# wyhuai/DDNM

Hardware: AMD Instinct MI355X
Metric: restored images/sec @256×256, 100 DDIM steps, 4×SR; 1/2/4/8 GPU (higher is better)
Workload: dtype f32 (3x3 convolutions: fp32 operands carried as hi + lo fp16 halves, three fp16 MFMA products per product, fp32 accumulate -- operand error 2^-22, measured closer to fp64 than the fp32 MFMA kernel; everything else fp32); 1 GPU; celeba_hq.yml SVD sr_bicubic 4x, sigma_y=0, eta=0.85, T_sampling=100, batch_size=8 per GPU (BASELINE configs[1]); global_batch=8, image=3x256x256, parallelism=dp1 (image sharding)

## Files before the change

ddnm_amd/_lib.py:

```python
import ctypes
import os
from ctypes import POINTER, Structure, c_char_p, c_float, c_int32, c_int64, c_uint8, c_uint32, c_void_p

_HERE = os.path.dirname(os.path.abspath(__file__))
LIB_PATH = os.path.join(_HERE, "libddnm_hip.so")

c_f32p = c_void_p


class ConvDesc(Structure):
    _fields_ = [
        ("src0", c_void_p), ("src1", c_void_p), ("weight", c_void_p), ("bias", c_void_p),
        ("badd", c_void_p), ("res", c_void_p), ("gn_scale", c_void_p), ("gn_shift", c_void_p),
        ("out", c_void_p),
        ("B", c_int32), ("Hin", c_int32), ("Win", c_int32),
        ("C0", c_int32), ("C1", c_int32), ("Cout", c_int32),
        ("ksize", c_int32), ("stride", c_int32), ("pad", c_int32),
        ("Ho", c_int32), ("Wo", c_int32),
        ("ups", c_int32), ("gn_silu", c_int32), ("out_nchw", c_int32),
        ("badd_stride", c_int32), ("tile", c_int32),
        ("workspace", c_void_p), ("workspace_floats", c_int64),
        ("res_ups", c_int32), ("src_f16", c_int32),
        ("stats_out", c_void_p),
        ("skip0", c_void_p), ("skip1", c_void_p), ("skip_weight", c_void_p),
# ... 32 lines not shown
        ("fin_gamma", c_void_p), ("fin_beta", c_void_p), ("fin_film", c_void_p),
        ("fin_scale", c_void_p), ("fin_shift", c_void_p),
        ("fin_eps", c_float), ("fin_film_stride", c_int32), ("fin_groups", c_int32), ("reserved2", c_int32),
    ]


class StepScalars(Structure):
    _fields_ = [("sqrt_1m_at", c_float), ("sqrt_at", c_float), ("sqrt_at_next", c_float),
                ("c1", c_float), ("c2", c_float), ("lam", c_float),
                ("rng_on", c_uint32), ("rng_seed_lo", c_uint32), ("rng_seed_hi", c_uint32), ("rng_iter", c_uint32),
                ("rng_image_base", c_uint32), ("reserved_rng", c_uint32)]


PROTOTYPES = {
    "ddnm_version": (c_int32, []),
    "ddnm_error_string": (c_char_p, [c_int32]),
    "ddnm_build_digest": (c_char_p, []),
    "ddnm_sizeof": (c_int32, [c_int32]),
    "ddnm_conv2d_f32": (c_int32, [POINTER(ConvDesc), c_void_p]),
    "ddnm_conv3x3_small_cout_f32": (c_int32, [POINTER(ConvDesc), c_void_p]),
    "ddnm_conv3x3_small_cout_f32_supported": (c_int32, [POINTER(ConvDesc)]),
    "ddnm_conv2d_f32_tile_n": (c_int32, [POINTER(ConvDesc)]),
    "ddnm_conv2d_f32_workspace_floats": (c_int64, [POINTER(ConvDesc)]),
    "ddnm_conv2d_f32_stats_tiles": (c_int32, [POINTER(ConvDesc)]),
    "ddnm_conv2d_f32_fuses_skip": (c_int32, [POINTER(ConvDesc)]),
    "ddnm_spectral_mix_f32": (c_int32, [c_void_p, c_void_p, c_void_p, c_int64, c_void_p, c_int64, c_float, c_float, c_float,
                                        c_float, c_int32, c_void_p]),
    "ddnm_hq_x0_f32": (c_int32, [c_void_p, c_void_p, c_int64, c_void_p, c_int32, c_int64, c_float, c_float, c_int32,
                                 c_void_p]),
    "ddnm_hq_project_f32": (c_int32, [c_void_p, c_void_p, c_void_p, c_void_p, c_int64, c_float, c_void_p]),
    "ddnm_copy_rect_f32": (c_int32, [c_void_p, c_int32, c_int32, c_int32, c_int32, c_void_p, c_int32, c_int32, c_int32,
                                     c_int32, c_int32, c_int32, c_int32, c_void_p]),
    "ddnm_hq_sample_f32": (c_int32, [c_void_p, c_void_p, c_void_p, c_void_p, c_void_p, c_int64, c_float, c_float, c_float,
                                     c_float, c_void_p]),
    "ddnm_patchify_f32": (c_int32, [c_void_p, c_void_p, c_int32, c_int32, c_int32, c_int32, c_void_p]),
    "ddnm_im2col3x3_f16": (c_int32, [c_void_p, c_void_p, c_void_p, c_void_p, c_void_p, c_int32, c_int32, c_int32, c_int32,
                                     c_int32, c_int32, c_void_p]),
    "ddnm_gn_apply_f16": (c_int32, [c_void_p, c_void_p, c_void_p, c_void_p, c_void_p, c_int32, c_int32, c_int32, c_int32,
                                    c_int32, c_void_p]),
    "ddnm_gn_finalize_tiles_f32": (c_int32, [c_void_p, c_int32, c_int32, c_void_p, c_int32, c_int32, c_void_p, c_void_p,
                                             c_int32, c_int32, c_int32, c_float, c_void_p, c_void_p, c_void_p, c_int32,
                                             c_void_p, c_void_p]),
    "ddnm_gn_finalize_tiles_amax_f32": (c_int32, [c_void_p, c_int32, c_int32, c_void_p, c_int32, c_int32, c_void_p, c_void_p,
                                                  c_int32, c_int32, c_int32, c_float, c_void_p, c_void_p, c_void_p, c_int32,
                                                  c_void_p, c_void_p, c_void_p]),
    "ddnm_amax_bound_f32": (c_int32, [c_void_p, c_int64, c_int32, c_void_p, c_int64, c_int32, c_void_p, c_int32, c_void_p]),
    "ddnm_conv3x3_f16_f32": (c_int32, [POINTER(ConvDesc), c_void_p]),
    "ddnm_conv3x3_f16_supported": (c_int32, [POINTER(ConvDesc)]),
    "ddnm_conv3x3_f16_workspace_floats": (c_int64, [POINTER(ConvDesc)]),
    "ddnm_conv3x3_f16_stats_tiles": (c_int32, [POINTER(ConvDesc)]),
    "ddnm_conv3x3_s16_f32": (c_int32, [POINTER(ConvDesc), c_void_p]),
    "ddnm_conv3x3_s16_supported": (c_int32, [POINTER(ConvDesc)]),
    "ddnm_conv3x3_s16_persistent": (c_int32, [POINTER(ConvDesc)]),
    "ddnm_conv3x3_s16_ups_subpixel_supported": (c_int32, [POINTER(ConvDesc)]),
    "ddnm_conv3x3_s16_workspace_floats": (c_int64, [POINTER(ConvDesc)]),
    "ddnm_conv3x3_s16_stats_tiles": (c_int32, [POINTER(ConvDesc)]),
    "ddnm_conv3x3_s16_act_scale": (c_float, []),
    "ddnm_conv_gather_s16_f32": (c_int32, [POINTER(ConvDesc), c_void_p]),
    "ddnm_conv_gather_s16_supported": (c_int32, [POINTER(ConvDesc)]),
    "ddnm_conv_gather_s16_workspace_floats": (c_int64, [POINTER(ConvDesc)]),
    "ddnm_conv_gather_s16_stats_tiles": (c_int32, [POINTER(ConvDesc)]),
    "ddnm_conv_gather_s16_gemm1x1": (c_int32, [POINTER(ConvDesc)]),
    "ddnm_conv_gather_s16_wslice": (c_int32, [POINTER(ConvDesc)]),
    "ddnm_conv16": (c_int32, [POINTER(Conv16Desc), c_void_p]),
    "ddnm_conv16_supported": (c_int32, [POINTER(Conv16Desc)]),
    "ddnm_conv16_fuses_fin": (c_int32, [POINTER(Conv16Desc)]),
    "ddnm_conv16_workspace_floats": (c_int64, [POINTER(Conv16Desc)]),
    "ddnm_conv16_stats_tiles": (c_int32, [POINTER(Conv16Desc)]),
    "ddnm_gn_apply_h16": (c_int32, [c_void_p, c_void_p, c_void_p, c_void_p, c_void_p, c_int32, c_int32, c_int32, c_int32,
                                    c_int32, c_int32, c_int32, c_void_p]),
    "ddnm_im2col3x3_h16": (c_int32, [c_void_p, c_void_p, c_void_p, c_void_p, c_void_p, c_int32, c_int32, c_int32, c_int32,
                                     c_int32, c_int32, c_void_p]),
    "ddnm_nchw_to_nhwc_h16": (c_int32, [c_void_p, c_void_p, c_int32, c_int32, c_int32, c_int32, c_void_p]),
    "ddnm_gn_stats_h16": (c_int32, [c_void_p, c_void_p, c_int32, c_int32, c_int32, c_int32, c_void_p]),
    "ddnm_attn16_d64": (c_int32, [c_void_p, c_void_p, c_int32, c_int32, c_int32, c_void_p]),
    "ddnm_conv1x1_f16_f32": (c_int32, [POINTER(ConvDesc), c_void_p]),
    "ddnm_conv1x1_f16_supported": (c_int32, [POINTER(ConvDesc)]),
    "ddnm_conv1x1_f16_workspace_floats": (c_int64, [POINTER(ConvDesc)]),
    "ddnm_conv1x1_f16_stats_tiles": (c_int32, [POINTER(ConvDesc)]),
    "ddnm_gn_stats_f32": (c_int32, [c_void_p, c_void_p, c_int32, c_int32, c_int32, c_int32, c_int32, c_void_p,
                                    c_int32, c_void_p]),
    "ddnm_gn_nchunk": (c_int32, [c_int32, c_int32]),
    "ddnm_gn_finalize_f32": (c_int32, [c_void_p, c_int32, c_void_p, c_void_p, c_int32, c_int32, c_int32, c_int32,
                                       c_float, c_void_p, c_void_p, c_void_p, c_int32, c_void_p, c_void_p]),
    "ddnm_bgemm_f32": (c_int32, [POINTER(GemmDesc), c_void_p]),
    "ddnm_gn_bwd_f32": (c_int32, [c_void_p, c_void_p, c_int32, c_void_p, c_void_p, c_void_p, c_int32, c_void_p, c_int32,
                                  c_int32, c_int32, c_int32, c_int32, c_int32, c_void_p, c_int32, c_void_p, c_void_p,
                                  c_void_p]),
    "ddnm_gn_bwd_nchunk": (c_int32, [c_int32, c_int32]),
    "ddnm_gn_bwd_h16": (c_int32, [c_void_p, c_void_p, c_int32, c_void_p, c_void_p, c_void_p, c_int32, c_void_p, c_int32,
                                  c_int32, c_int32, c_int32, c_int32, c_int32, c_void_p, c_int32, c_void_p, c_void_p,
                                  c_void_p]),
    "ddnm_pool_tokens_h16": (c_int32, [c_void_p, c_void_p, c_void_p, c_void_p, c_void_p, c_int32, c_int32, c_int32,
                                       c_void_p]),
    "ddnm_pool_tokens_bwd_h16": (c_int32, [c_void_p, c_void_p, c_int32, c_int32, c_int32, c_void_p]),
    "ddnm_attn16_d64_lse": (c_int32, [c_void_p, c_void_p, c_void_p, c_int32, c_int32, c_int32, c_void_p]),
    "ddnm_attn16_d64_bwd": (c_int32, [c_void_p, c_void_p, c_void_p, c_void_p, c_void_p, c_void_p, c_int32, c_int32,
                                      c_int32, c_void_p]),
    "ddnm_softmax_bwd_rows_f32": (c_int32, [c_void_p, c_void_p, c_int64, c_int32, c_int32, c_float, c_void_p]),
    "ddnm_pool_tokens_f32": (c_int32, [c_void_p, c_void_p, c_void_p, c_void_p, c_void_p, c_int32, c_int32, c_int32,
                                       c_void_p]),
    "ddnm_pool_attn_fwd_f32": (c_int32, [c_void_p, c_void_p, c_void_p, c_int32, c_int32, c_int32, c_int32, c_void_p]),
    "ddnm_pool_attn_bwd_f32": (c_int32, [c_void_p, c_void_p, c_void_p, c_void_p, c_int32, c_int32, c_int32, c_int32,
                                         c_void_p]),
    "ddnm_pool_tokens_bwd_f32": (c_int32, [c_void_p, c_void_p, c_int32, c_int32, c_int32, c_void_p]),
    "ddnm_logsoftmax_grad_f32": (c_int32, [c_void_p, c_void_p, c_void_p, c_int32, c_int32, c_void_p]),
# ... 170 lines not shown
```

ddnm_amd/build.py:

```python
import hashlib
import os
import shutil
import subprocess
import sys

HERE = os.path.dirname(os.path.abspath(__file__))
CSRC = os.path.join(HERE, "csrc")
LIB = os.path.join(HERE, "libddnm_hip.so")
STAMP = os.path.join(HERE, ".libddnm_hip.stamp")
OBJ = os.path.join(HERE, "_obj")
SOURCES = ["conv_igemm_f32.hip", "conv_igemm_f16.hip", "conv_s16_persist.hip", "conv_s16_subpixel.hip", "conv_gather_s16.hip", "conv1x1_s16.hip", "conv_s16_wslice.hip", "conv_small_f32.hip", "conv1x1_f16.hip", "conv16.hip", "act16.hip", "attn16.hip", "attn_d512.hip", "attn16_bwd.hip", "gemm_f32.hip", "groupnorm.hip", "misc.hip", "ddnm_step.hip", "fwht.hip", "backward.hip", "metrics.hip"]
FLAGS = ["--offload-arch=gfx950", "-O3", "-std=c++17", "-fPIC", "-shared", "-Wall", "-Wno-unused-function"]


def _hipcc():
    for c in (os.environ.get("HIPCC"), shutil.which("hipcc"), "/opt/rocm/bin/hipcc"):
        if c and os.path.exists(c):
            return c
    raise RuntimeError("hipcc not found (set HIPCC)")


def _digest():
    h = hashlib.sha256()
    for f in sorted(os.listdir(CSRC)) + ["../../include/ddnm_hip.h"]:
        with open(os.path.join(CSRC, f), "rb") as fh:
            h.update(f.encode() + fh.read())
    h.update(" ".join(FLAGS).encode())
    return h.hexdigest()


LAST_BUILD = {"compiled": False}


def build(force=False, verbose=False):
    dig = _digest()
    LAST_BUILD["compiled"] = False
    if not force and os.path.exists(LIB) and os.path.exists(STAMP) and open(STAMP).read() == dig:
        return LIB
    LAST_BUILD["compiled"] = True
    tmp = LIB + f".tmp{os.getpid()}"
    os.makedirs(OBJ, exist_ok=True)
    hh = hashlib.sha256()
    for f in sorted(os.listdir(CSRC)) + ["../../include/ddnm_hip.h"]:
        if f.endswith(".h"):
            with open(os.path.join(CSRC, f), "rb") as fh:
                hh.update(f.encode() + fh.read())
    hh.update(" ".join(FLAGS).encode())
    cflags = [f for f in FLAGS if f != "-shared"]
    jobs, objs = [], []
    for s in SOURCES:
        h = hashlib.sha256(hh.digest())
        with open(os.path.join(CSRC, s), "rb") as fh:
            h.update(fh.read())
        extra = [f'-DDDNM_BUILD_DIGEST="{dig}"'] if s == "misc.hip" else []
        h.update(" ".join(extra).encode())
        obj = os.path.join(OBJ, f"{s}.{h.hexdigest()[:16]}.o")
        objs.append(obj)
        if force or not os.path.exists(obj):
            jobs.append((s, [_hipcc()] + cflags + extra + ["-c", os.path.join(CSRC, s), "-o", obj + f".tmp{os.getpid()}"], obj))
    if jobs:
        from concurrent.futures import ThreadPoolExecutor

        def run(job):
            s, cmd, obj = job
# ... 34 lines not shown
```

ddnm_amd/csrc/conv_common.h:

```cpp
#pragma once
#include "common.h"

struct ConvArgs {
    ddnm_conv_desc d;
    int Cin, ntaps, Hs, Ws;
    int m_tiles, n_tiles;
    int tiles_x;
    int TW, TW_log2;
    int ksplit;
    float* ws;
};

static inline bool conv_operand_offsets_fit(const ddnm_conv_desc* d) {
    const int64_t px = (int64_t)d->B * (d->ups ? d->Hin / 2 : d->Hin) * (d->ups ? d->Win / 2 : d->Win);
    const int64_t cmax = d->C0 > d->C1 ? d->C0 : d->C1;
    return px * cmax * (d->src_f16 ? 2 : 4) < (int64_t)1 << 31;
}
static inline bool conv_sizes_addressable(const ddnm_conv_desc* d) {
    const int64_t lim = (int64_t)1 << 31;
    const int64_t out_el = (int64_t)d->B * d->Ho * d->Wo * d->Cout;
    const int64_t cout_pad = ((int64_t)d->Cout + 127) / 128 * 128;
    const int64_t w_b = cout_pad * d->ksize * d->ksize * ((int64_t)d->C0 + d->C1) * 4;
    const int64_t sk_el = (int64_t)d->B * d->Ho * d->Wo * (d->SC0 > d->SC1 ? d->SC0 : d->SC1);
    return out_el < lim && conv_operand_offsets_fit(d) && w_b < lim && sk_el < lim;
}

bool conv3x3_s16_persist_eligible(const ConvArgs& p);
int conv3x3_s16_persist_launch(const ConvArgs& p, hipStream_t s);
bool conv3x3_s16_ups_subpixel_ok(const ddnm_conv_desc* d);
int conv3x3_s16_ups_subpixel_run(const ddnm_conv_desc* d, hipStream_t s);
bool conv1x1_s16_routes(const ddnm_conv_desc* d, int plan_ksplit, int plan_bm);
int conv1x1_s16_launch(const ddnm_conv_desc* d, int plan_ksplit, int plan_bm, int run_ksplit, hipStream_t s);
bool conv3x3_s16_wslice_routes(const ddnm_conv_desc* d, int plan_ksplit, int plan_bm);
int conv3x3_s16_wslice_launch(const ddnm_conv_desc* d, int ksplit, hipStream_t s);
int conv_persist_grid_cus();

struct TileMap {
    int img, ty0, tx0, th_unused, TW, TW_log2, flat_base, Wo;
    bool two_d;
    __device__ __forceinline__ void pixel(int r, int& oy, int& ox) const {
        if (two_d) {
            oy = ty0 + (r >> TW_log2);
            ox = tx0 + (r & (TW - 1));
        } else {
            const int pix = flat_base + r;
            oy = pix / Wo;
            ox = pix - oy * Wo;
        }
    }
};

template <int BM>
__device__ __forceinline__ TileMap make_tilemap(const ConvArgs& p, int m_tile) {
    TileMap t;
    const int HWo = p.d.Ho * p.d.Wo;
    const int per_img = HWo / BM;
    t.img = m_tile / per_img;
    const int t_in_img = m_tile - t.img * per_img;
    t.TW = p.TW;
    t.TW_log2 = p.TW_log2;
    t.Wo = p.d.Wo;
    t.two_d = p.tiles_x != 0;
    if (t.two_d) {
        const int ty = t_in_img / p.tiles_x, tx = t_in_img - ty * p.tiles_x;
        t.ty0 = ty * (BM >> p.TW_log2);
        t.tx0 = tx << p.TW_log2;
        t.flat_base = 0;
    } else {
        t.ty0 = t.tx0 = 0;
        t.flat_base = t_in_img * BM;
    }
    return t;
}

template <int WM, int WN, int MT, int NT, bool RES_ALL_UPFRONT = false>
__device__ __forceinline__ void conv_epilogue(const ConvArgs& p, const TileMap& tm, int n_tile, int m_tile, int slice,
                                              f32x16 (&acc)[MT][NT], float* lds, const float acc_scale = 1.f) {
    constexpr int BN = WN * NT * 32;
    const ddnm_conv_desc& d = p.d;
    const int lane = threadIdx.x & 63, wave = threadIdx.x >> 6;
    const int wm = wave / WN, wn = wave % WN;
    const int ncol = lane & 31, rsel = 4 * (lane >> 5);
    const bool partial = p.ksplit > 1;
    float* __restrict__ ws = partial ? p.ws + (size_t)slice * d.B * d.Ho * d.Wo * d.Cout : nullptr;
    const float* __restrict__ res = d.res;
    float* __restrict__ out = d.out;
    const bool want_stats = d.stats_out != nullptr && !partial;
// ... 314 lines not shown
```

ddnm_amd/csrc/conv_igemm_f16.hip:

```cpp
#include "s16_tile.h"

constexpr int KC16 = 64;
constexpr int F16_BM = 256;
constexpr int F16_KS_TARGET = 256;
constexpr int LDH = KC16 + 8;

template <int WM, int WN, int MT, int NT, bool SRC16, bool SPLIT = false, bool ASCALE = false>
__global__ __launch_bounds__(WM * WN * 64, 1) void conv3x3_halo_f16_kernel(const ConvArgs p) {
    static_assert(!(SPLIT && SRC16), "the split form reads fp32 activations");
    static_assert(SPLIT || !ASCALE, "operand scaling belongs to the split form");
    constexpr int NTHREADS = WM * WN * 64;
    constexpr int BM = WM * MT * 32, BN = WN * NT * 32;
    constexpr int MAXH = BM == 512 ? 612 : (BM == 256 ? 340 : (BM == 128 ? 204 : 136));
    constexpr int KCH = SPLIT ? KC16 / 2 : KC16;
    constexpr int WE = SPLIT ? 2 : 1;
    constexpr int HVEC = SRC16 ? 8 : 4;
    constexpr int HCOLS = KCH / HVEC;
    constexpr int HROWS_PER_PASS = NTHREADS / HCOLS;
    constexpr int HR = (MAXH + HROWS_PER_PASS - 1) / HROWS_PER_PASS;
    static_assert(KC16 == 64, "an LDS weight row is 128 bytes");
    constexpr int BCOLS = 8;
    constexpr int BROWS_PER_PASS = NTHREADS / BCOLS;
    constexpr int BR = BN / BROWS_PER_PASS;
    static_assert(BR >= 1 && BN % BROWS_PER_PASS == 0, "weight tile / thread mapping");
// ... 281 lines not shown
    int tw = 32;
    while (tw > 8 && (d->Wo % tw || d->Ho % (pl->BM / tw))) tw >>= 1;
    if (d->Wo % tw || d->Ho % (pl->BM / tw)) return false;
    pl->TW = tw;
    pl->TW_log2 = tw == 32 ? 5 : (tw == 16 ? 4 : 3);
    pl->tiles_x = d->Wo / tw;
    const long tiles = (long)d->B * (HWo / pl->BM) * (d->Cout / 128);
    int ks = 1;
    const int nchunks = Cin / kch;
    if (tiles < 192) {
        ks = (int)((F16_KS_TARGET + tiles - 1) / tiles);
        if (ks > nchunks) ks = nchunks;
        if (ks > 16) ks = 16;
    }
    pl->ksplit = ks;
    return true;
}

extern "C" int ddnm_conv3x3_f16_supported(const ddnm_conv_desc* d) {
    PlanF16 pl;
    return d && plan_f16(d, &pl) ? 1 : 0;
}

extern "C" int64_t ddnm_conv3x3_f16_workspace_floats(const ddnm_conv_desc* d) {
    PlanF16 pl;
    if (!d || !plan_f16(d, &pl)) return DDNM_E_SHAPE;
    return conv_slab_floats(d, pl.ksplit);
}

extern "C" int ddnm_conv3x3_f16_stats_tiles(const ddnm_conv_desc* d) {
    PlanF16 pl;
    if (!d || !plan_f16(d, &pl)) return DDNM_E_SHAPE;
    return conv_stats_tiles(d, pl.ksplit, pl.BM);
}

static int run_f16(const ddnm_conv_desc* d, void* stream, bool split) {
    const int kch = split ? KC16 / 2 : KC16;
    if (!d) return DDNM_E_BADARG;
    if (split && (d->src_f16 || !(d->acc_scale > 0.f))) return DDNM_E_BADARG;
    if (split && !d->amax_in && (!d->gn_scale || d->skip0)) return DDNM_E_BADARG;
    if (int e = conv_check_desc(d)) return e;
    if (d->src_f16 && d->gn_scale) return DDNM_E_BADARG;
    if (int e = conv_check_gn_ups(d)) return e;
    PlanF16 pl;
    if (!plan_f16(d, &pl, kch)) return DDNM_E_SHAPE;
    if (d->skip0) {
        if (d->ups || !d->skip_weight || d->SC0 <= 0 || d->SC0 % kch || d->SC1 % kch || (d->SC1 > 0 && !d->skip1))
            return DDNM_E_SHAPE;
    }
    if ((pl.ksplit = conv_run_ksplit(d, pl.ksplit)) < 0) return pl.ksplit;
    const ConvArgs p = conv_args(*d, pl.BM, d->Cout / 128, pl.TW, pl.TW_log2, pl.tiles_x, 9, pl.ksplit);
    hipStream_t s = (hipStream_t)stream;
    if (split && !(d->flags & DDNM_CONV_ONE_TILE) && conv3x3_s16_persist_eligible(p)) return conv3x3_s16_persist_launch(p, s);
    const dim3 grid(p.m_tiles * p.n_tiles, pl.ksplit);
    if (split && d->amax_in) { DDNM_LAUNCH((conv3x3_halo_f16_kernel<4, 2, 2, 2, false, true, true>), grid, dim3(512), 0, s, p); }
    else if (split) { DDNM_LAUNCH((conv3x3_halo_f16_kernel<4, 2, 2, 2, false, true>), grid, dim3(512), 0, s, p); }
    else if (d->src_f16) { DDNM_LAUNCH((conv3x3_halo_f16_kernel<4, 2, 2, 2, true>), grid, dim3(512), 0, s, p); }
    else { DDNM_LAUNCH((conv3x3_halo_f16_kernel<4, 2, 2, 2, false>), grid, dim3(512), 0, s, p); }
    if (pl.ksplit > 1) return launch_splitk_reduce(p, s);
    return 0;
}

extern "C" int ddnm_conv3x3_f16_f32(const ddnm_conv_desc* d, void* stream) { return run_f16(d, stream, false); }

extern "C" int ddnm_conv3x3_s16_f32(const ddnm_conv_desc* d, void* stream) {
    if (d && (d->flags & DDNM_CONV_UPS_SUBPIXEL)) return conv3x3_s16_ups_subpixel_run(d, (hipStream_t)stream);
    return run_f16(d, stream, true);
}

extern "C" int ddnm_conv3x3_s16_ups_subpixel_supported(const ddnm_conv_desc* d) { return conv3x3_s16_ups_subpixel_ok(d) ? 1 : 0; }

extern "C" float ddnm_conv3x3_s16_act_scale(void) { return DDNM_S16_ASCALE; }

extern "C" int ddnm_conv3x3_s16_persistent(const ddnm_conv_desc* d) {
    PlanF16 pl;
    if (!d || (d->flags & DDNM_CONV_UPS_SUBPIXEL) || d->src_f16 || (d->flags & DDNM_CONV_ONE_TILE) || !plan_f16(d, &pl, KC16 / 2) || pl.ksplit != 1) return 0;
    return conv3x3_s16_persist_eligible(conv_args(*d, pl.BM, d->Cout / 128, pl.TW, pl.TW_log2, pl.tiles_x, 9, 1)) ? 1 : 0;
}

extern "C" int ddnm_conv3x3_s16_supported(const ddnm_conv_desc* d) {
    PlanF16 pl;
    return d && !d->src_f16 && plan_f16(d, &pl, KC16 / 2) ? 1 : 0;
}

extern "C" int64_t ddnm_conv3x3_s16_workspace_floats(const ddnm_conv_desc* d) {
    PlanF16 pl;
    if (d && (d->flags & DDNM_CONV_UPS_SUBPIXEL)) return conv3x3_s16_ups_subpixel_ok(d) ? 0 : DDNM_E_SHAPE;
    if (!d || !plan_f16(d, &pl, KC16 / 2)) return DDNM_E_SHAPE;
    return conv_slab_floats(d, pl.ksplit);
}

extern "C" int ddnm_conv3x3_s16_stats_tiles(const ddnm_conv_desc* d) {
    PlanF16 pl;
    if (d && (d->flags & DDNM_CONV_UPS_SUBPIXEL)) return conv3x3_s16_ups_subpixel_ok(d) ? d->Ho * d->Wo / 256 : DDNM_E_SHAPE;
    if (!d || !plan_f16(d, &pl, KC16 / 2)) return DDNM_E_SHAPE;
    return conv_stats_tiles(d, pl.ksplit, pl.BM);
}
```

ddnm_amd/ops.py:

```python
import ctypes
import math
from typing import Callable, NamedTuple, Optional

import numpy as np
import torch

from . import _lib
from ._lib import Conv16Desc, ConvDesc, GemmDesc, StepScalars, check


def _p(t):
    return None if t is None else t.data_ptr()


def _stream():
    return torch.cuda.current_stream().cuda_stream


def _f32c(t, name):
    if t.dtype != torch.float32 or not t.is_contiguous() or not t.is_cuda:
        raise ValueError(f"{name}: expected a contiguous float32 device tensor, got {t.dtype} "
                         f"contiguous={t.is_contiguous()} device={t.device}")
    return t

# ... 93 lines not shown


def pack_skip_weight(w, f16=False):
    p = pack_conv_weight(w).reshape(-1, w.shape[1]).contiguous()
    return p.to(torch.float16) if f16 else p


def pack_conv_weight_f16(w, cin_pad=None):
    return pack_conv_weight(w, cin_pad=cin_pad).to(torch.float16).contiguous()


def s16_weight_scale(*ws):
    m = max(float(w.abs().max()) for w in ws)
    if not (m > 0.0) or not math.isfinite(m):
        return 1.0
    return 2.0 ** (13 - math.floor(math.log2(m)))


def s16_weight_row_bound(scale, *ws):
    num = den = None
    for w in ws:
        v = w.detach().to(torch.float64)
        v = (v.flatten(0, 2) if v.dim() == 6 else v).flatten(1).abs() * float(scale)
        eps = torch.where(v == 0, torch.zeros_like(v), torch.where(v < 0.25, torch.full_like(v, 2.0 ** -25), v * 2.0 ** -22))
        n, d_ = eps.sum(1), v.sum(1)
        num, den = (n, d_) if num is None else (num + n, den + d_)
    live = den > 0
    if not bool(live.any()):
        return 0.0
    return float((num[live] / den[live]).max())


S16_WEIGHT_ROW_LIMIT = 2.0 ** -21


def pack_conv_weight_s16(w, scale):
    p = pack_conv_weight(w) * float(scale)
    cp, taps, cin = p.shape
    if cin % 32:
        raise ValueError("split packing needs Cin % 32 == 0")
    hi = p.to(torch.float16)
    lo = (p - hi.float()).to(torch.float16)
    hi, lo = hi.view(cp, taps, cin // 32, 1, 32), lo.view(cp, taps, cin // 32, 1, 32)
    return torch.cat([hi, lo], 3).contiguous()


def upsample_phase_weights(w):
    w = w.detach().to(torch.float64)
    sel = torch.tensor([[[1, 0, 0], [0, 1, 1]], [[1, 1, 0], [0, 0, 1]]], dtype=torch.float64, device=w.device)
    return torch.einsum("pak,qbl,oikl->pqoiab", sel, sel, w)


UPS_SUBPIXEL = 2


def pack_upsample_conv_weight_s16(w, scale):
    cout, cin = w.shape[:2]
    if tuple(w.shape[2:]) != (3, 3) or cin % 32 or cout % 64:
        raise ValueError("phase packing needs 3x3 weights, Cin % 32 == 0 and Cout % 64 == 0")
    wp = upsample_phase_weights(w) * float(scale)
    wp = wp.reshape(2, 2, cout // 64, 64, cin, 4).permute(2, 0, 1, 3, 5, 4).reshape(4 * cout, 4, cin)
    hi = wp.to(torch.float16)
    lo = (wp - hi.double()).to(torch.float16)
    hi, lo = hi.view(4 * cout, 4, cin // 32, 1, 32), lo.view(4 * cout, 4, cin // 32, 1, 32)
    return torch.cat([hi, lo], 3).contiguous()


def upsample_weight_s16(w):
    sc = s16_weight_scale(upsample_phase_weights(w))
    return (pack_upsample_conv_weight_s16(w, sc), sc, None)


def conv_runs_ups_subpixel(B, H, W, cin, cout):
    d = _shape_desc(B, 2 * H, 2 * W, cin, cout)
    d.ups, d.flags = 1, UPS_SUBPIXEL
    return _lib.lib().ddnm_conv3x3_s16_ups_subpixel_supported(ctypes.byref(d)) == 1


def conv_runs_s16(B, H, W, cin, cout, ups=False):
    return _lib.lib().ddnm_conv3x3_s16_supported(ctypes.byref(_shape_desc(B, H, W, cin, cout))) == 1


def conv_runs_s16_gather(B, H, W, cin, cout, ksize=3, stride=1):
    if _NO_S16_GATHER:
        return False
    return _lib.lib().ddnm_conv_gather_s16_supported(ctypes.byref(_shape_desc(B, H, W, cin, cout, ksize, stride))) == 1


_S16_ACT_SCALE = None


def _s16_act_scale():
    global _S16_ACT_SCALE
    if _S16_ACT_SCALE is None:
        _S16_ACT_SCALE = float(_lib.lib().ddnm_conv3x3_s16_act_scale())
    return _S16_ACT_SCALE


def conv_runs_f16(B, H, W, cin, cout, ksize=3):
    L = _lib.lib()
    d = _shape_desc(B, H, W, cin, cout, ksize)
    return (L.ddnm_conv3x3_f16_supported if ksize == 3 else L.ddnm_conv1x1_f16_supported)(ctypes.byref(d)) == 1


_f16_scratch_buf = {}

# ... 110 lines not shown
            if g is not None:
                return CONV_FAMILIES["f16_1x1"], g, None
    elif d.ksize == 1 and not d.skip0:
        g = _desc_copy(d, gn_scale=None, gn_shift=None)
        if L.ddnm_conv1x1_f16_supported(ctypes.byref(g)) == 1:
            fam, launch = CONV_FAMILIES["f16_1x1"], g
    if fam.pack == "f16" and gn is not None and (fam.name == "f16_1x1" or d.Cout >= _F16_PREPASS_MIN_COUT):
        launch = _f16_gn_prepass(L, d, src0, src1, gn_silu)
    return fam, launch, gn


def _select_conv_family(L, d, src0, src1, gn, gn_silu, weight_s16, weight_f16):
    q, fused = ctypes.byref(d), bool(d.skip0)
    if (d.out_nchw and d.Cout <= 4 and not fused and weight_f16 is None
            and L.ddnm_conv3x3_small_cout_f32_supported(q) == 1):
        return CONV_FAMILIES["small_cout"], d, gn
    if weight_f16 is not None:
        return _select_f16(L, d, src0, src1, gn, gn_silu)
    if weight_s16 is not None:
        if d.flags == UPS_SUBPIXEL:
            return CONV_FAMILIES["s16_subpixel"], d, gn
        if (d.ksize == 3 and d.stride == 1
                and (not fused or (weight_s16[2] is not None and gn is not None and d.SC0 % 32 == 0 and d.SC1 % 32 == 0))
                and L.ddnm_conv3x3_s16_supported(q) == 1):
            return CONV_FAMILIES["s16"], d, gn
        if not fused and not _NO_S16_GATHER and L.ddnm_conv_gather_s16_supported(q) == 1:
            return CONV_FAMILIES["s16_gather"], d, gn
    return CONV_FAMILIES["f32"], d, gn


def _launch_conv(L, fam, d, out, emit_stats, record):
    stats, tiles = None, 0
    if emit_stats and fam.stats_tiles is not None:
        tiles = getattr(L, fam.stats_tiles)(ctypes.byref(d))
        if tiles < 0 and fam.strict:
            check(tiles, fam.stats_tiles)
        if tiles > 0:
            stats = torch.empty(d.B * tiles * d.Cout * 2, dtype=torch.float32, device=out.device)
            d.stats_out = stats.data_ptr()
    if fam.workspace_floats is not None:
        need = getattr(L, fam.workspace_floats)(ctypes.byref(d))
        if need < 0 and fam.strict:
            check(int(need), fam.workspace_floats)
        if need > 0:
            ws = _conv_workspace(out.device, need)
            d.workspace, d.workspace_floats = ws.data_ptr(), ws.numel()
    _launch(getattr(L, fam.run), d, fam.label, record)
    return Act(out, stats, tiles)


def conv2d(src0, weight, cout, ksize, *, src1=None, bias=None, badd=None, badd_stride=0, res=None, res_ups=False,
           gn=None, gn_silu=True, stride=1, pad=None, ups=False, out=None, out_nchw=False, out_hw=None, tile=0,
           emit_stats=False, weight_f16=None, skip=None, skip_weight=None, skip_weight_f16=None, weight_s16=None,
           raw_amax=None, one_tile=False, ups_subpixel=False):
    a_src0, a_src1 = src0, src1
    src0, src1, res = tensor_of(src0), tensor_of(src1), tensor_of(res)
    B, Hs, Ws, C0 = src0.shape
    C1 = 0 if src1 is None else src1.shape[3]
    Hin, Win = (2 * Hs, 2 * Ws) if ups else (Hs, Ws)
    if pad is None:
        pad = ksize // 2
    Ho, Wo = (Hin // stride, Win // stride) if out_hw is None else out_hw
    if out is None:
        shape = (B, cout, Ho, Wo) if out_nchw else (B, Ho, Wo, cout)
        out = torch.empty(shape, dtype=torch.float32, device=src0.device)
    d = ConvDesc()
    d.src0, d.src1, d.weight = _p(_f32c(src0, "src0")), _p(src1), _p(_f32c(weight, "weight"))
    d.bias, d.badd, d.res = _p(bias), _p(badd), _p(res)
    d.gn_scale, d.gn_shift = (None, None) if gn is None else (_p(gn[0]), _p(gn[1]))
    d.out = _p(out)
    d.B, d.Hin, d.Win, d.C0, d.C1, d.Cout = B, Hin, Win, C0, C1, cout
    d.ksize, d.stride, d.pad, d.Ho, d.Wo = ksize, stride, pad, Ho, Wo
    d.ups, d.gn_silu, d.out_nchw = int(ups), int(gn_silu), int(out_nchw)
    d.badd_stride, d.tile, d.res_ups = badd_stride, tile, int(res_ups)
    d.flags = UPS_SUBPIXEL if ups_subpixel else (1 if (one_tile or FORCE_ONE_TILE) else 0)
    if skip is not None:
        s0, s1 = tensor_of(skip[0]), tensor_of(skip[1])
        d.skip0, d.skip1 = _p(s0), _p(s1)
        d.SC0, d.SC1 = s0.shape[3], (0 if s1 is None else s1.shape[3])
    L = _lib.lib()
    if ups_subpixel and (not ups or weight_s16 is None or weight_f16 is not None or skip is not None
                         or L.ddnm_conv3x3_s16_ups_subpixel_supported(ctypes.byref(d)) != 1):
        raise ValueError(f"ups_subpixel: launch (B={B}, {Hs}x{Ws} -> {Ho}x{Wo}, Cin={C0 + C1}, Cout={cout}) does not "
                         "qualify (ddnm_conv3x3_s16_ups_subpixel_supported)")
    fam, d, gn = _select_conv_family(L, d, src0, src1, gn, gn_silu, weight_s16, weight_f16)
    if fam.pack == "s16":
        d.weight = weight_s16[0].data_ptr()
        d.acc_scale = 1.0 / (float(weight_s16[1]) * _s16_act_scale())
        if gn is None or skip is not None:
            if raw_amax is None:
                raw_amax = amax_bound(*skip) if skip is not None else amax_bound(a_src0, a_src1)
            d.amax_in = raw_amax.data_ptr()
    elif fam.pack == "f16":
        d.weight = weight_f16.data_ptr()
    if skip is not None:
        if fam.pack == "f16" and skip_weight_f16 is None:
            raise ValueError("fp16 launch with a fused shortcut needs skip_weight_f16")
        d.skip_weight = _p(skip_weight_f16 if fam.pack == "f16" else weight_s16[2] if fam.pack == "s16" else skip_weight)

    def record():
        flops = 2.0 * B * Ho * Wo * cout * (ksize * ksize * (C0 + C1) + d.SC0 + d.SC1)
        if ups_subpixel:
            flops *= 16.0 / 36.0
        return fam.variant(L, d), flops, (B, Ho, Wo, C0 + C1, cout, ksize, stride, int(ups), d.SC0 + d.SC1, gn is not None,
                                          res is not None)
    act = _launch_conv(L, fam, d, out, emit_stats and not _NO_FUSED_GN, record)
    if _S16_CHECK and fam.pack == "s16" and not bool(torch.isfinite(out).all()):
        raise FloatingPointError(f"split-fp16 launch produced non-finite values (B={B}, {Hin}x{Win}, Cin={C0 + C1}, "
                                 f"Cout={cout}, k={ksize}): an operand left fp16 range; DDNM_CONV_F32=mfma32 selects the "
                                 "all-fp32 engine")
    return act if emit_stats else out


CONV16_COUT_ALIGN = 256


def _f16c(t, name):
    if t.dtype != torch.float16 or not t.is_contiguous() or not t.is_cuda:
        raise ValueError(f"{name}: expected a contiguous float16 device tensor, got {t.dtype} "
                         f"contiguous={t.is_contiguous()} device={t.device}")
    return t


def pack_conv_weight16(w, cin_pad=None):
    if w.dim() == 2:
        w = w[:, :, None, None]
    cout, cin, kh, kw = w.shape
    cin_pad = cin if cin_pad is None else cin_pad
# ... 589 lines not shown
```

include/ddnm_hip.h:

```cpp
#ifndef DDNM_HIP_H
#define DDNM_HIP_H

#include <stdint.h>

#ifdef __cplusplus
extern "C" {
#endif

#define DDNM_E_BADARG (-1)
#define DDNM_E_SHAPE (-2)

int ddnm_version(void);
const char* ddnm_build_digest(void);
int ddnm_sizeof(int which);
const char* ddnm_error_string(int code);

typedef struct ddnm_conv_desc {
    const float* src0;
    const float* src1;
    const float* weight;
    const float* bias;
    const float* badd;
    const float* res;
    const float* gn_scale;
    const float* gn_shift;
    float* out;
    int32_t B, Hin, Win;
    int32_t C0, C1;
    int32_t Cout;
    int32_t ksize;
    int32_t stride;
    int32_t pad;
    int32_t Ho, Wo;
    int32_t ups;
    int32_t gn_silu;
    int32_t out_nchw;
    int32_t badd_stride;
    int32_t tile;
    float* workspace;
    int64_t workspace_floats;
    int32_t res_ups;
    int32_t src_f16;
    float* stats_out;
    const float* skip0;
    const float* skip1;
    const float* skip_weight;
    int32_t SC0, SC1;
    float acc_scale;
    int32_t flags;
    const float* amax_in;
} ddnm_conv_desc;

#define DDNM_CONV_ONE_TILE 1
#define DDNM_CONV_UPS_SUBPIXEL 2
#define DDNM_CONV_GEMM1X1 4
#define DDNM_AMAX_N 32

int ddnm_conv2d_f32(const ddnm_conv_desc* d, void* stream);
int ddnm_conv2d_f32_tile_n(const ddnm_conv_desc* d);
int64_t ddnm_conv2d_f32_workspace_floats(const ddnm_conv_desc* d);
int ddnm_conv2d_f32_stats_tiles(const ddnm_conv_desc* d);
int ddnm_conv2d_f32_fuses_skip(const ddnm_conv_desc* d);

int ddnm_conv3x3_small_cout_f32(const ddnm_conv_desc* d, void* stream);
int ddnm_conv3x3_small_cout_f32_supported(const ddnm_conv_desc* d);

int ddnm_conv3x3_f16_f32(const ddnm_conv_desc* d, void* stream);
int ddnm_conv3x3_f16_supported(const ddnm_conv_desc* d);
int64_t ddnm_conv3x3_f16_workspace_floats(const ddnm_conv_desc* d);
int ddnm_conv3x3_f16_stats_tiles(const ddnm_conv_desc* d);

int ddnm_conv3x3_s16_f32(const ddnm_conv_desc* d, void* stream);
int ddnm_conv3x3_s16_supported(const ddnm_conv_desc* d);
int ddnm_conv3x3_s16_persistent(const ddnm_conv_desc* d);
int64_t ddnm_conv3x3_s16_workspace_floats(const ddnm_conv_desc* d);
int ddnm_conv3x3_s16_stats_tiles(const ddnm_conv_desc* d);
int ddnm_conv3x3_s16_ups_subpixel_supported(const ddnm_conv_desc* d);
float ddnm_conv3x3_s16_act_scale(void);

int ddnm_conv_gather_s16_f32(const ddnm_conv_desc* d, void* stream);
int ddnm_conv_gather_s16_supported(const ddnm_conv_desc* d);
int64_t ddnm_conv_gather_s16_workspace_floats(const ddnm_conv_desc* d);
int ddnm_conv_gather_s16_stats_tiles(const ddnm_conv_desc* d);
int ddnm_conv_gather_s16_gemm1x1(const ddnm_conv_desc* d);
int ddnm_conv_gather_s16_wslice(const ddnm_conv_desc* d);

int ddnm_conv1x1_f16_f32(const ddnm_conv_desc* d, void* stream);
int ddnm_conv1x1_f16_supported(const ddnm_conv_desc* d);
int64_t ddnm_conv1x1_f16_workspace_floats(const ddnm_conv_desc* d);
int ddnm_conv1x1_f16_stats_tiles(const ddnm_conv_desc* d);

typedef struct ddnm_conv16_desc {
    const void* src;
    const void* weight;
    const float* bias;
    const void* res;
    const void* skip0;
    const void* skip1;
    const void* skip_weight;
    void* out;
    float* stats_out;
    float* workspace;
    int64_t workspace_floats;
    int32_t B, H, W;
    int32_t Cin, Cout;
    int32_t ksize;
    int32_t ups, res_ups;
    int32_t SC0, SC1;
    const void* src1;
    const float* gn_scale;
    const float* gn_shift;
    int32_t C0;
    int32_t gn_silu;
    int32_t out_nchw_f32;
    int32_t reserved;
    const float* fin_gamma;
    const float* fin_beta;
    const float* fin_film;
    float* fin_scale;
    float* fin_shift;
    float fin_eps;
    int32_t fin_film_stride;
    int32_t fin_groups;
    int32_t reserved2;
} ddnm_conv16_desc;

int ddnm_conv16(const ddnm_conv16_desc* d, void* stream);
int ddnm_conv16_fuses_fin(const ddnm_conv16_desc* d);
int ddnm_conv16_supported(const ddnm_conv16_desc* d);
int64_t ddnm_conv16_workspace_floats(const ddnm_conv16_desc* d);
// ... 289 lines not shown
```

Measured before the change: 6.427 images/sec.

## Add full-K s16 3x3 conv kernel replacing split-K for small-Cin layers

Adds a new 3x3 conv kernel that walks the whole input-channel range inside one workgroup instead of launching split-K slices. It keeps a 9-tap weight ring in LDS with a double-buffered halo, and interleaves MFMA with LDS reads through sched_group_barrier. The epilogue applies bias, residual and group-norm tile stats directly, so the split-K workspace and reduction pass go away. It routes automatically when Cin<=160, or when Cin<=256 with enough workgroups, and the persistent kernel still takes precedence. Per-slice accumulators are folded in a fixed order to keep results identical to split-K summation, at the cost of less parallelism per layer.

```diff
diff --git a/ddnm_amd/_lib.py b/ddnm_amd/_lib.py
--- a/ddnm_amd/_lib.py
+++ b/ddnm_amd/_lib.py
@@ -108,6 +108,7 @@
     "ddnm_conv3x3_s16_f32": (c_int32, [POINTER(ConvDesc), c_void_p]),
     "ddnm_conv3x3_s16_supported": (c_int32, [POINTER(ConvDesc)]),
     "ddnm_conv3x3_s16_persistent": (c_int32, [POINTER(ConvDesc)]),
+    "ddnm_conv3x3_s16_fullk": (c_int32, [POINTER(ConvDesc)]),
     "ddnm_conv3x3_s16_ups_subpixel_supported": (c_int32, [POINTER(ConvDesc)]),
     "ddnm_conv3x3_s16_workspace_floats": (c_int64, [POINTER(ConvDesc)]),
     "ddnm_conv3x3_s16_stats_tiles": (c_int32, [POINTER(ConvDesc)]),
diff --git a/ddnm_amd/build.py b/ddnm_amd/build.py
--- a/ddnm_amd/build.py
+++ b/ddnm_amd/build.py
@@ -9,7 +9,7 @@
 LIB = os.path.join(HERE, "libddnm_hip.so")
 STAMP = os.path.join(HERE, ".libddnm_hip.stamp")
 OBJ = os.path.join(HERE, "_obj")
-SOURCES = ["conv_igemm_f32.hip", "conv_igemm_f16.hip", "conv_s16_persist.hip", "conv_s16_subpixel.hip", "conv_gather_s16.hip", "conv1x1_s16.hip", "conv_s16_wslice.hip", "conv_small_f32.hip", "conv1x1_f16.hip", "conv16.hip", "act16.hip", "attn16.hip", "attn_d512.hip", "attn16_bwd.hip", "gemm_f32.hip", "groupnorm.hip", "misc.hip", "ddnm_step.hip", "fwht.hip", "backward.hip", "metrics.hip"]
+SOURCES = ["conv_igemm_f32.hip", "conv_igemm_f16.hip", "conv_s16_persist.hip", "conv_s16_subpixel.hip", "conv_gather_s16.hip", "conv1x1_s16.hip", "conv_s16_wslice.hip", "conv_s16_fullk.hip", "conv_small_f32.hip", "conv1x1_f16.hip", "conv16.hip", "act16.hip", "attn16.hip", "attn_d512.hip", "attn16_bwd.hip", "gemm_f32.hip", "groupnorm.hip", "misc.hip", "ddnm_step.hip", "fwht.hip", "backward.hip", "metrics.hip"]
 FLAGS = ["--offload-arch=gfx950", "-O3", "-std=c++17", "-fPIC", "-shared", "-Wall", "-Wno-unused-function"]
 
 
diff --git a/ddnm_amd/csrc/conv_common.h b/ddnm_amd/csrc/conv_common.h
--- a/ddnm_amd/csrc/conv_common.h
+++ b/ddnm_amd/csrc/conv_common.h
@@ -33,6 +33,9 @@
 int conv1x1_s16_launch(const ddnm_conv_desc* d, int plan_ksplit, int plan_bm, int run_ksplit, hipStream_t s);
 bool conv3x3_s16_wslice_routes(const ddnm_conv_desc* d, int plan_ksplit, int plan_bm);
 int conv3x3_s16_wslice_launch(const ddnm_conv_desc* d, int ksplit, hipStream_t s);
+bool conv3x3_s16_fullk_has_form(const ddnm_conv_desc* d, int plan_tw, int ksplit);
+bool conv3x3_s16_fullk_routes(const ddnm_conv_desc* d, int plan_tw, int ksplit);
+int conv3x3_s16_fullk_launch(const ddnm_conv_desc* d, int ksplit, hipStream_t s);
 int conv_persist_grid_cus();
 
 struct TileMap {
diff --git a/ddnm_amd/csrc/conv_igemm_f16.hip b/ddnm_amd/csrc/conv_igemm_f16.hip
--- a/ddnm_amd/csrc/conv_igemm_f16.hip
+++ b/ddnm_amd/csrc/conv_igemm_f16.hip
@@ -357,6 +357,7 @@
     const ConvArgs p = conv_args(*d, pl.BM, d->Cout / 128, pl.TW, pl.TW_log2, pl.tiles_x, 9, pl.ksplit);
     hipStream_t s = (hipStream_t)stream;
     if (split && !(d->flags & DDNM_CONV_ONE_TILE) && conv3x3_s16_persist_eligible(p)) return conv3x3_s16_persist_launch(p, s);
+    if (split && !(d->flags & DDNM_CONV_ONE_TILE) && conv3x3_s16_fullk_routes(d, pl.TW, pl.ksplit)) return conv3x3_s16_fullk_launch(d, pl.ksplit, s);
     const dim3 grid(p.m_tiles * p.n_tiles, pl.ksplit);
     if (split && d->amax_in) { DDNM_LAUNCH((conv3x3_halo_f16_kernel<4, 2, 2, 2, false, true, true>), grid, dim3(512), 0, s, p); }
     else if (split) { DDNM_LAUNCH((conv3x3_halo_f16_kernel<4, 2, 2, 2, false, true>), grid, dim3(512), 0, s, p); }
@@ -383,6 +384,12 @@
     return conv3x3_s16_persist_eligible(conv_args(*d, pl.BM, d->Cout / 128, pl.TW, pl.TW_log2, pl.tiles_x, 9, 1)) ? 1 : 0;
 }
 
+extern "C" int ddnm_conv3x3_s16_fullk(const ddnm_conv_desc* d) {
+    PlanF16 pl;
+    if (!d || (d->flags & DDNM_CONV_UPS_SUBPIXEL) || d->src_f16 || !plan_f16(d, &pl, KC16 / 2)) return DDNM_E_SHAPE;
+    return !(d->flags & DDNM_CONV_ONE_TILE) && conv3x3_s16_fullk_routes(d, pl.TW, pl.ksplit) ? 1 : 0;
+}
+
 extern "C" int ddnm_conv3x3_s16_supported(const ddnm_conv_desc* d) {
     PlanF16 pl;
     return d && !d->src_f16 && plan_f16(d, &pl, KC16 / 2) ? 1 : 0;
diff --git a/ddnm_amd/csrc/conv_s16_fullk.hip b/ddnm_amd/csrc/conv_s16_fullk.hip
--- /dev/null
+++ b/ddnm_amd/csrc/conv_s16_fullk.hip
@@ -0,0 +1,288 @@
+#include "s16_tile.h"
+
+typedef unsigned u32x2 __attribute__((ext_vector_type(2)));
+
+constexpr int FK_WM = 4, FK_WN = 2, FK_WAVES = FK_WM * FK_WN, FK_NTHREADS = FK_WAVES * 64;
+constexpr int FK_TH = 4, FK_TW = 32;
+constexpr int FK_BM = FK_TH * FK_TW, FK_BN = FK_WN * 32;
+constexpr int FK_HWD = FK_TW + 2, FK_HROWS = (FK_TH + 2) * FK_HWD;
+constexpr int FK_HPP = FK_NTHREADS / S16_HCOLS;
+constexpr int FK_HR = (FK_HROWS + FK_HPP - 1) / FK_HPP;
+constexpr int FK_HALO = FK_HROWS * S16_LDH;
+constexpr int FK_WTILE = FK_BN * 128;
+constexpr int FK_NWL = 9;
+constexpr int FK_RING = 9;
+constexpr int FK_LDS = FK_NWL * FK_WTILE + 2 * FK_HALO * 2;
+static_assert(FK_WTILE == FK_WAVES * 1024, "one 16-byte request per lane and weight tile");
+static_assert(FK_LDS <= 160 * 1024, "LDS of one CU");
+
+template <int P, int ROWS>
+__device__ __forceinline__ void fk_tile_stats_rows(const float (&p)[P], float& s, float& q) {
+#pragma clang fp contract(off)
+    s = q = 0.f;
+#pragma unroll
+    for (int r = 0; r < (ROWS < P ? ROWS : P); ++r) {
+        float sr = p[r], qr = p[r] * p[r];
+#pragma unroll
+        for (int pp = r + ROWS; pp < P; pp += ROWS) {
+            sr = sr + p[pp];
+            qr = __builtin_fmaf(p[pp], p[pp], qr);
+        }
+        s = r == 0 ? sr : s + sr;
+        q = r == 0 ? qr : q + qr;
+    }
+}
+__device__ __forceinline__ void fk_oct_stats(const float (&p)[8], int rows, float& s, float& q) {
+    switch (rows) {
+        case 1: fk_tile_stats_rows<8, 1>(p, s, q); break;
+        case 2: fk_tile_stats_rows<8, 2>(p, s, q); break;
+        case 3: fk_tile_stats_rows<8, 3>(p, s, q); break;
+        case 4: fk_tile_stats_rows<8, 4>(p, s, q); break;
+        case 5: fk_tile_stats_rows<8, 5>(p, s, q); break;
+        case 6: fk_tile_stats_rows<8, 6>(p, s, q); break;
+        case 7: fk_tile_stats_rows<8, 7>(p, s, q); break;
+        default: fk_tile_stats_rows<8, 8>(p, s, q); break;
+    }
+}
+
+__global__ __launch_bounds__(FK_NTHREADS) void conv_s16_fullk_kernel(const ConvArgs p, const int stat_px) {
+    __shared__ __attribute__((aligned(1024))) char lds_all[FK_LDS];
+    char* const Bs = lds_all;
+    _Float16* const Hs = reinterpret_cast<_Float16*>(lds_all + FK_NWL * FK_WTILE);
+
+    const ddnm_conv_desc& d = p.d;
+    const int tid = threadIdx.x, lane = tid & 63;
+    const int wave = __builtin_amdgcn_readfirstlane(tid >> 6);
+    const int wm = wave / FK_WN, wn = wave % FK_WN;
+    const int tile_id = xcd_swizzle(blockIdx.x, gridDim.x);
+    const int n_tile = tile_id % p.n_tiles, m_tile = tile_id / p.n_tiles;
+    const int per_img = p.tiles_x * (d.Ho / FK_TH);
+    const int img = m_tile / per_img, t_in_img = m_tile - img * per_img;
+    const int ty0 = (t_in_img / p.tiles_x) * FK_TH, tx0 = (t_in_img % p.tiles_x) * FK_TW;
+    float ascale, inv_ascale;
+    s16_operand_scale(d.amax_in, img, d.gn_scale != nullptr, ascale, inv_ascale);
+
+    const int lrow = lane >> 3, lpiece = lane & 7;
+    const unsigned w_rowlen = 9u * (unsigned)p.Cin * 4u;
+    const __amdgpu_buffer_rsrc_t r_w = __builtin_amdgcn_make_buffer_rsrc(
+        const_cast<void*>(reinterpret_cast<const void*>(d.weight)), 0, (unsigned)d.Cout * w_rowlen, 0x00020000);
+    const unsigned w_voff = S16_W_LANE(n_tile * FK_BN + wave * 8 + lrow, w_rowlen, lpiece, S16_W_SWZ(wave, lrow));
+    auto load_w = [&](int chunk, int tap) {
+        return __builtin_amdgcn_raw_buffer_load_b128(r_w, w_voff, ((unsigned)tap * (unsigned)p.Cin + (unsigned)chunk * S16_KCH) * 4u, 0);
+    };
+    char* const w_dst = Bs + wave * 1024 + lane * 16;
+    auto stage_w = [&](int buf, const u32x4& v) { *reinterpret_cast<u32x4*>(w_dst + buf * FK_WTILE) = v; };
+    const int b_frag = S16_B_FRAG(wn * 32, lane);
+
+    const bool has_gn = d.gn_scale != nullptr;
+    const int hc = tid & (S16_HCOLS - 1), prow = tid / S16_HCOLS;
+    const __amdgpu_buffer_rsrc_t r_s0 = __builtin_amdgcn_make_buffer_rsrc(
+        const_cast<float*>(d.src0), 0, (unsigned)d.B * d.Hin * d.Win * d.C0 * 4u, 0x00020000);
+    const __amdgpu_buffer_rsrc_t r_s1 = __builtin_amdgcn_make_buffer_rsrc(
+        const_cast<float*>(d.C1 > 0 ? d.src1 : d.src0), 0, (unsigned)d.B * d.Hin * d.Win * (d.C1 > 0 ? d.C1 : d.C0) * 4u, 0x00020000);
+    const unsigned gn_bytes = has_gn ? (unsigned)d.B * p.Cin * 4u : 0u;
+    const __amdgpu_buffer_rsrc_t r_gsc = __builtin_amdgcn_make_buffer_rsrc(
+        const_cast<float*>(has_gn ? d.gn_scale : d.src0), 0, gn_bytes, 0x00020000);
+    const __amdgpu_buffer_rsrc_t r_gsh = __builtin_amdgcn_make_buffer_rsrc(
+        const_cast<float*>(has_gn ? d.gn_shift : d.src0), 0, gn_bytes, 0x00020000);
+    const unsigned gn_voff = ((unsigned)img * p.Cin + hc * 4) * 4u;
+    int hpix[FK_HR];
+#pragma unroll
+    for (int i = 0; i < FK_HR; ++i) {
+        const int r = prow + FK_HPP * i;
+        const int hy = r / FK_HWD, hx = r - hy * FK_HWD;
+        const int iy = ty0 + hy - 1, ix = tx0 + hx - 1;
+        const bool ok = r < FK_HROWS && (unsigned)iy < (unsigned)d.Hin && (unsigned)ix < (unsigned)d.Win;
+        hpix[i] = ok ? (img * d.Hin + iy) * d.Win + ix : -1;
+    }
+    struct Halo {
+        f32x4 v[FK_HR], gsc, gsh;
+    };
+    auto prefetch_a = [&](int chunk, Halo& h, bool live) {
+        const int cb = chunk * S16_KCH;
+        const bool first = cb < d.C0;
+        const unsigned cs = first ? d.C0 : d.C1, coff = first ? cb : cb - d.C0;
+        const __amdgpu_buffer_rsrc_t r_s = first ? r_s0 : r_s1;
+#pragma unroll
+        for (int i = 0; i < FK_HR; ++i) {
+            const unsigned vo = (hpix[i] >= 0 && live) ? ((unsigned)hpix[i] * cs + hc * 4) * 4u : S16_OOB;
+            h.v[i] = __builtin_bit_cast(f32x4, __builtin_amdgcn_raw_buffer_load_b128(r_s, vo, coff * 4u, 0));
+        }
+        h.gsc = __builtin_bit_cast(f32x4, __builtin_amdgcn_raw_buffer_load_b128(r_gsc, gn_voff, (unsigned)cb * 4u, 0));
+        h.gsh = __builtin_bit_cast(f32x4, __builtin_amdgcn_raw_buffer_load_b128(r_gsh, gn_voff, (unsigned)cb * 4u, 0));
+    };
+    auto stage_a = [&](const Halo& h, int hbuf) {
+#pragma unroll
+        for (int i = 0; i < FK_HR; ++i) {
+            f32x4 v = h.v[i];
+            if (has_gn && hpix[i] >= 0) v = gn_act(v, h.gsc, h.gsh, d.gn_silu);
+            const int r = prow + FK_HPP * i;
+            if (r < FK_HROWS) split_store(&Hs[hbuf * FK_HALO + r * S16_LDH + hc * 4], v, ascale);
+        }
+    };
+
+    f32x16 acc[1][1], total;
+#pragma unroll
+    for (int r = 0; r < 16; ++r) acc[0][0][r] = total[r] = 0.f;
+
+    const int a_off[1] = {(wm * FK_HWD + (lane & 31)) * S16_LDH + (lane >> 5) * 8};
+
+    const int nchunks = p.Cin / S16_KCH, ksplit = p.ksplit;
+    int slice = 0, slice_end = nchunks / ksplit;
+    {
+        Halo h;
+        u32x4 w[FK_RING];
+        prefetch_a(0, h, true);
+#pragma unroll
+        for (int t = 0; t < FK_RING; ++t) w[t] = load_w(0, t);
+        stage_a(h, 0);
+#pragma unroll
+        for (int k = 0; k < 3; ++k) stage_w(k, w[k]);
+        int hb = 0;
+        for (int c = 0; c < nchunks; ++c) {
+            const bool more = c + 1 < nchunks;
+            const int cn = more ? c + 1 : c;
+            const _Float16* const a = Hs + hb * FK_HALO;
+#pragma unroll
+            for (int g = 0; g < 3; ++g) {
+                asm volatile("s_waitcnt lgkmcnt(0)" ::: "memory");
+                __builtin_amdgcn_s_barrier();
+                asm volatile("" ::: "memory");
+                if (g == 0) {
+                    prefetch_a(cn, h, more);
+                    __builtin_amdgcn_sched_barrier(0);
+                }
+#pragma unroll
+                for (int k = 0; k < 3; ++k) w[3 * g + k] = load_w(cn, 3 * g + k);
+                __builtin_amdgcn_sched_barrier(0);
+                const int gn = (g + 1) % 3;
+#pragma unroll
+                for (int k = 0; k < 3; ++k) stage_w(3 * gn + k, w[3 * gn + k]);
+                if (g == 2) stage_a(h, hb ^ 1);
+                __builtin_amdgcn_sched_barrier(0);
+#pragma unroll
+                for (int k = 0; k < 3; ++k)
+                    s16_mfma_tile<1, 1>(acc, a, a_off, (g * FK_HWD + k) * S16_LDH, Bs + (3 * g + k) * FK_WTILE, b_frag);
+                __builtin_amdgcn_sched_group_barrier(0x100, 8, 0);
+#pragma unroll
+                for (int i = 0; i < 4; ++i) {
+                    __builtin_amdgcn_sched_group_barrier(0x008, 1, 0);
+                    __builtin_amdgcn_sched_group_barrier(0x100, 2, 0);
+                    __builtin_amdgcn_sched_group_barrier(0x008, 1, 0);
+                    __builtin_amdgcn_sched_group_barrier(0x100, 1, 0);
+                    __builtin_amdgcn_sched_group_barrier(0x008, 1, 0);
+                    __builtin_amdgcn_sched_group_barrier(0x100, 1, 0);
+                }
+                __builtin_amdgcn_sched_group_barrier(0x008, 6, 0);
+                __builtin_amdgcn_sched_barrier(0);
+            }
+            hb ^= 1;
+            const bool fold = c + 1 == slice_end;
+#pragma unroll
+            for (int r = 0; r < 16; ++r) {
+                const float t = total[r] + acc[0][0][r];
+                total[r] = fold ? t : total[r];
+                acc[0][0][r] = fold ? 0.f : acc[0][0][r];
+            }
+            slice += fold ? 1 : 0;
+            slice_end = (int)((unsigned)(nchunks * (slice + 1)) / (unsigned)ksplit);
+        }
+    }
+
+    const float epi = d.acc_scale * inv_ascale;
+    const unsigned n = (unsigned)(n_tile * FK_BN + wn * 32 + (lane & 31));
+    const unsigned out_bytes = (unsigned)d.B * d.Ho * d.Wo * d.Cout * 4u;
+    const __amdgpu_buffer_rsrc_t r_out = __builtin_amdgcn_make_buffer_rsrc(d.out, 0, out_bytes, 0x00020000);
+    const __amdgpu_buffer_rsrc_t r_res = __builtin_amdgcn_make_buffer_rsrc(
+        const_cast<float*>(d.res ? d.res : d.out), 0, d.res ? out_bytes : 0u, 0x00020000);
+    const __amdgpu_buffer_rsrc_t r_bias = __builtin_amdgcn_make_buffer_rsrc(
+        const_cast<float*>(d.bias ? d.bias : d.out), 0, d.bias ? (unsigned)d.Cout * 4u : 0u, 0x00020000);
+    const __amdgpu_buffer_rsrc_t r_badd = __builtin_amdgcn_make_buffer_rsrc(
+        const_cast<float*>(d.badd ? d.badd : d.out), 0, d.badd ? ((unsigned)(d.B - 1) * d.badd_stride + d.Cout) * 4u : 0u, 0x00020000);
+    const float bias = __uint_as_float(__builtin_amdgcn_raw_buffer_load_b32(r_bias, n * 4u, 0, 0));
+    const float badd = __uint_as_float(__builtin_amdgcn_raw_buffer_load_b32(r_badd, ((unsigned)img * d.badd_stride + n) * 4u, 0, 0));
+    const unsigned pix_row = (unsigned)((img * d.Ho + ty0 + wm) * d.Wo + tx0) + 4u * (lane >> 5);
+    unsigned o[16];
+    float rv[16];
+#pragma unroll
+    for (int r = 0; r < 16; ++r) {
+        o[r] = ((pix_row + (r & 3) + 8 * (r >> 2)) * (unsigned)d.Cout + n) * 4u;
+        rv[r] = __uint_as_float(__builtin_amdgcn_raw_buffer_load_b32(r_res, o[r], 0, 0));
+    }
+    float v[16];
+#pragma unroll
+    for (int r = 0; r < 16; ++r) {
+        if (d.stats_out) {
+            float add = 0.f;
+            if (d.bias) add = add + bias;
+            if (d.badd) add = add + badd;
+            v[r] = add + total[r] * epi;
+            if (d.res) v[r] = v[r] + rv[r];
+        } else {
+            v[r] = total[r] * epi;
+            if (d.bias) v[r] = v[r] + bias;
+            if (d.badd) v[r] = v[r] + badd;
+            if (d.res) v[r] = v[r] + rv[r];
+        }
+        __builtin_amdgcn_raw_buffer_store_b32(__float_as_uint(v[r]), r_out, o[r], 0, 0);
+    }
+    if (d.stats_out) {
+        const int rows = 256 / (d.Cout >> 2);
+        const __amdgpu_buffer_rsrc_t r_st = __builtin_amdgcn_make_buffer_rsrc(
+            d.stats_out, 0, (unsigned)d.B * d.Ho * d.Wo / (unsigned)stat_px * d.Cout * 8u, 0x00020000);
+#pragma unroll
+        for (int g = 0; g < 4; ++g) {
+            const unsigned pix0 = pix_row + 8 * g;
+            float cs, cq;
+            unsigned so;
+            if (stat_px == 4) {
+                s16_quad_stats(v[4 * g], v[4 * g + 1], v[4 * g + 2], v[4 * g + 3], rows, cs, cq);
+                so = ((pix0 >> 2) * (unsigned)d.Cout + n) * 8u;
+            } else {
+                float q[8];
+#pragma unroll
+                for (int e = 0; e < 4; ++e) {
+                    const float mine = v[4 * g + e], other = __shfl_xor(mine, 32);
+                    q[e] = lane < 32 ? mine : other;
+                    q[4 + e] = lane < 32 ? other : mine;
+                }
+                fk_oct_stats(q, rows, cs, cq);
+                so = lane < 32 ? ((pix0 >> 3) * (unsigned)d.Cout + n) * 8u : S16_OOB;
+            }
+            const u32x2 st = {__float_as_uint(cs), __float_as_uint(cq)};
+            __builtin_amdgcn_raw_buffer_store_b64(st, r_st, so, 0, 0);
+        }
+    }
+}
+
+static int fullk_stat_px(const ddnm_conv_desc* d) {
+    const int tpi = splitk_stats_tiles(d);
+    if (tpi <= 0) return 0;
+    const int hw = d->Ho * d->Wo;
+    return hw == 4 * tpi ? 4 : (hw == 8 * tpi ? 8 : 0);
+}
+bool conv3x3_s16_fullk_routes(const ddnm_conv_desc* d, int plan_tw, int ksplit) {
+    if (!conv3x3_s16_fullk_has_form(d, plan_tw, ksplit)) return false;
+    if (d->flags & DDNM_CONV_FULLK) return true;
+    const int cin = d->C0 + d->C1;
+    const long workgroups = (long)d->B * (d->Ho * d->Wo / FK_BM) * (d->Cout / FK_BN);
+    return cin <= 160 || (cin <= 256 && workgroups >= 64);
+}
+
+bool conv3x3_s16_fullk_has_form(const ddnm_conv_desc* d, int plan_tw, int ksplit) {
+    if (d->ksize != 3 || d->stride != 1 || d->pad != 1 || d->ups || d->res_ups || d->out_nchw || d->skip0) return false;
+    if (d->Ho != d->Hin || d->Wo != d->Win || plan_tw != FK_TW || d->Wo % FK_TW || d->Ho % FK_TH) return false;
+    if (d->C0 <= 0 || d->C0 % S16_KCH || d->C1 % S16_KCH || d->Cout % FK_BN) return false;
+    if (ksplit < 2 || ksplit > (d->C0 + d->C1) / S16_KCH) return false;
+    if (d->stats_out && fullk_stat_px(d) == 0) return false;
+    if ((int64_t)d->B * d->Ho * d->Wo * d->Cout * 4 >= (int64_t)1 << 31) return false;
+    if (d->badd && ((int64_t)(d->B - 1) * d->badd_stride + d->Cout) * 4 >= (int64_t)1 << 31) return false;
+    return true;
+}
+
+int conv3x3_s16_fullk_launch(const ddnm_conv_desc* d, int ksplit, hipStream_t s) {
+    const ConvArgs p = conv_args(*d, FK_BM, d->Cout / FK_BN, FK_TW, 5, d->Wo / FK_TW, 9, ksplit);
+    const int stat_px = d->stats_out ? fullk_stat_px(d) : 0;
+    DDNM_LAUNCH(conv_s16_fullk_kernel, dim3(p.m_tiles * p.n_tiles), dim3(FK_NTHREADS), 0, s, p, stat_px);
+    return 0;
+}
diff --git a/ddnm_amd/ops.py b/ddnm_amd/ops.py
--- a/ddnm_amd/ops.py
+++ b/ddnm_amd/ops.py
@@ -169,6 +169,7 @@
 
 
 UPS_SUBPIXEL = 2
+FULLK = 8
 
 
 def pack_upsample_conv_weight_s16(w, scale):
@@ -385,7 +386,7 @@
 def conv2d(src0, weight, cout, ksize, *, src1=None, bias=None, badd=None, badd_stride=0, res=None, res_ups=False,
            gn=None, gn_silu=True, stride=1, pad=None, ups=False, out=None, out_nchw=False, out_hw=None, tile=0,
            emit_stats=False, weight_f16=None, skip=None, skip_weight=None, skip_weight_f16=None, weight_s16=None,
-           raw_amax=None, one_tile=False, ups_subpixel=False):
+           raw_amax=None, one_tile=False, ups_subpixel=False, full_k=False):
     a_src0, a_src1 = src0, src1
     src0, src1, res = tensor_of(src0), tensor_of(src1), tensor_of(res)
     B, Hs, Ws, C0 = src0.shape
@@ -406,7 +407,7 @@
     d.ksize, d.stride, d.pad, d.Ho, d.Wo = ksize, stride, pad, Ho, Wo
     d.ups, d.gn_silu, d.out_nchw = int(ups), int(gn_silu), int(out_nchw)
     d.badd_stride, d.tile, d.res_ups = badd_stride, tile, int(res_ups)
-    d.flags = UPS_SUBPIXEL if ups_subpixel else (1 if (one_tile or FORCE_ONE_TILE) else 0)
+    d.flags = UPS_SUBPIXEL if ups_subpixel else (1 if (one_tile or FORCE_ONE_TILE) else (FULLK if full_k else 0))
     if skip is not None:
         s0, s1 = tensor_of(skip[0]), tensor_of(skip[1])
         d.skip0, d.skip1 = _p(s0), _p(s1)
diff --git a/include/ddnm_hip.h b/include/ddnm_hip.h
--- a/include/ddnm_hip.h
+++ b/include/ddnm_hip.h
@@ -54,6 +54,7 @@
 #define DDNM_CONV_ONE_TILE 1
 #define DDNM_CONV_UPS_SUBPIXEL 2
 #define DDNM_CONV_GEMM1X1 4
+#define DDNM_CONV_FULLK 8
 #define DDNM_AMAX_N 32
 
 int ddnm_conv2d_f32(const ddnm_conv_desc* d, void* stream);
@@ -76,6 +77,7 @@
 int64_t ddnm_conv3x3_s16_workspace_floats(const ddnm_conv_desc* d);
 int ddnm_conv3x3_s16_stats_tiles(const ddnm_conv_desc* d);
 int ddnm_conv3x3_s16_ups_subpixel_supported(const ddnm_conv_desc* d);
+int ddnm_conv3x3_s16_fullk(const ddnm_conv_desc* d);
 float ddnm_conv3x3_s16_act_scale(void);
 
 int ddnm_conv_gather_s16_f32(const ddnm_conv_desc* d, void* stream);
```

Result: no change. 6.437 images/sec, median of 6 (+0.2%).
